# bmerry/mlsgpu

Hardware: AMD Instinct MI355X
Metric: Mvoxels/s evaluated+triangulated (higher is better)
Workload: dtype f32; 1 GPU; cfg3: 512^3 grid, 50000000 splats (uniform), 27 buckets of <= 171 cells per side, octree+MLS+MC end-to-end; bucket_splats_total=52997386, mesh_memory_mb=4096, device_workers=3, batch=8, marching_group=2, mls_variant=culled+matrix-prefilter, counts_cover=the whole cloud

## Files before the change

mlsgpu_amd/csrc/octree.hip:

```cpp
#include "common.hpp"
#include "primitives.hpp"

#include <cstdlib>

using namespace mlsgpu;

struct LevelOffsets
{
    uint32_t v[32];
};

struct mlsgpu_tree
{
    mlsgpu_ctx *ctx = nullptr;
    uint64_t maxLevels = 0, maxSplats = 0;
    uint64_t maxStart = 0, commandsSize = 0;
    uint32_t numLevels = 0;
    DeviceArray<int32_t> dStart, dJumpPos, dCommands;
    DeviceArray<uint32_t> dKeysA, dKeysB, dValsA, dValsB;
    DeviceArray<uint32_t> dHist, dTileSums, dNumEntries;
    DeviceArray<uint32_t> dNodeCounts, dNodeBase;
    DeviceArray<uint32_t> dDigitBase;
    DeviceArray<U3> dNodeTiles;
    HostMailbox entryBox;
    DeviceArray<uint8_t> dSlotMasks;
    DeviceArray<uint64_t> dEntryNotes;
    mlsgpu_splat *dSplats = nullptr;
    bool mutate = true;

    mlsgpu_tree(uint64_t maxLevels, uint64_t maxSplats) : maxLevels(maxLevels), maxSplats(maxSplats)
    {
        maxStart = (uint64_t(1) << (3 * maxLevels)) / 7;
        commandsSize = maxSplats * 8 + std::min(maxStart, 8 * maxSplats) * 2;
    }
    ~mlsgpu_tree() { entryBox.destroy(); }

    template<typename Each>
    int buffers(Each each)
    {
        const uint64_t entries = maxSplats * 8;
        const uint64_t histElems = sortHistElems(entries);
        PROPAGATE(each(dStart, maxStart));
        PROPAGATE(each(dJumpPos, maxStart));
        PROPAGATE(each(dCommands, commandsSize));
        PROPAGATE(each(dKeysA, entries));
        PROPAGATE(each(dKeysB, entries));
        PROPAGATE(each(dValsA, entries));
        PROPAGATE(each(dValsB, entries));
        PROPAGATE(each(dHist, histElems));
        PROPAGATE(each(dTileSums, (uint64_t) scanTiles(std::max(histElems, entries)) + 1));
        PROPAGATE(each(dNumEntries, 1));
        PROPAGATE(each(dSlotMasks, maxSplats));
        PROPAGATE(each(dEntryNotes, maxSplats));
        PROPAGATE(each(dNodeCounts, maxStart));
        PROPAGATE(each(dNodeBase, maxStart));
        PROPAGATE(each(dDigitBase, 257));
        PROPAGATE(each(dNodeTiles, (uint64_t) scanTiles(maxStart) + 1));
        return MLSGPU_OK;
    }
};

namespace
{

__device__ __forceinline__ uint32_t spread3(uint32_t v)
{
    v &= 0x3FFu;
    v = (v | (v << 16)) & 0x030000FFu;
    v = (v | (v << 8)) & 0x0300F00Fu;
    v = (v | (v << 4)) & 0x030C30C3u;
    v = (v | (v << 2)) & 0x09249249u;
    return v;
}
__device__ __forceinline__ uint32_t spreadNext(uint32_t s)
{
    return ((s | ~0x09249249u) + 1u) & 0x09249249u;
}
__device__ __forceinline__ uint32_t makeCode(int x, int y, int z)
{
    return spread3((uint32_t) x) | (spread3((uint32_t) y) << 1) | (spread3((uint32_t) z) << 2);
}
static_assert((0x09249249u & 7u) == 1u, "spread3 keeps bit 0 of a coordinate in bit 0");

__device__ uint32_t makeCodeLoop(int x, int y, int z)
{
    uint32_t ans = 0, scale = 1;
    y <<= 1;
    z <<= 2;
    while (x != 0 || y != 0 || z != 0)
    {
        uint32_t bits = (x & 1) | (y & 2) | (z & 4);
        ans += bits * scale;
        scale <<= 3;
        x >>= 1; y >>= 1; z >>= 1;
    }
    return ans;
}

__device__ __forceinline__ int levelShift(int lox, int loy, int loz, int hix, int hiy, int hiz)
{
    int big = max(max(hix - lox, hiy - loy), hiz - loz);
    return big > 1 ? 32 - __clz(big - 1) : 0;
}

__device__ __forceinline__ float pointBoxDist2(float px, float py, float pz, float lx, float ly, float lz,
                                                float hx, float hy, float hz)
{
    float dx = fmaxf(lx, fminf(hx, px)) - px;
    float dy = fmaxf(ly, fminf(hy, py)) - py;
    float dz = fmaxf(lz, fminf(hz, pz)) - pz;
    return dx * dx + dy * dy + dz * dz;
}

__device__ __forceinline__ int floorToInt(float v)
{
    float f = floorf(v);
    if (!(f > -2147483648.0f)) return INT32_MIN;
    if (!(f < 2147483648.0f)) return INT32_MAX;
    return (int) f;
}

struct EntryParams
{
    mlsgpu_splat *splats;
    int bx, by, bz;
    LevelOffsets levelOffsets;
    int minShift, maxShift;
    uint32_t firstSplat;
    uint32_t mutate;
};

struct EntryPlace
{
    int shift, ilx, ily, ilz;
};

__device__ __forceinline__ uint32_t splatEntries(const EntryParams &P, const float4 pr, uint32_t k[8], EntryPlace *place = nullptr)
{
    const int lox = floorToInt(pr.x - pr.w), loy = floorToInt(pr.y - pr.w), loz = floorToInt(pr.z - pr.w);
    const int hix = floorToInt(pr.x + pr.w), hiy = floorToInt(pr.y + pr.w), hiz = floorToInt(pr.z + pr.w);
    int shift = levelShift(lox, loy, loz, hix, hiy, hiz);
    shift = min(max(shift, P.minShift), P.maxShift);
    const int ilx = max(lox - P.bx, 0) >> shift;
    const int ily = max(loy - P.by, 0) >> shift;
    const int ilz = max(loz - P.bz, 0) >> shift;
    float radius2 = pr.w * pr.w;
    radius2 *= 1.00001f;
    const uint32_t levelOffset = P.levelOffsets.v[shift];
    const int bound = 1 << (P.maxShift - shift);
    if (place != nullptr)
        *place = EntryPlace{shift, ilx, ily, ilz};
    uint32_t mask = 0;
#pragma unroll
    for (int o = 0; o < 8; o++)
    {
        const int ax = ilx + (o & 1), ay = ily + ((o >> 1) & 1), az = ilz + (o >> 2);
        const int blx = (int) ((uint32_t) ax << shift) + P.bx, bhx = (int) ((uint32_t) (ax + 1) << shift) + P.bx;
        const int bly = (int) ((uint32_t) ay << shift) + P.by, bhy = (int) ((uint32_t) (ay + 1) << shift) + P.by;
        const int blz = (int) ((uint32_t) az << shift) + P.bz, bhz = (int) ((uint32_t) (az + 1) << shift) + P.bz;
        bool isect = pointBoxDist2(pr.x, pr.y, pr.z, (float) blx, (float) bly, (float) blz,
                                   (float) bhx, (float) bhy, (float) bhz) < radius2;
        isect = isect && ax < bound && ay < bound && az < bound;
        k[o] = makeCode(ax, ay, az) + levelOffset;
        mask |= (isect ? 1u : 0u) << o;
    }
    return mask;
}

struct EntryCountIn
{
    EntryParams P;
    uint8_t *slotMasks;
    __device__ __forceinline__ uint32_t operator()(uint64_t i) const
    {
        const float4 pr = reinterpret_cast<const float4 *>(P.splats + (i + P.firstSplat))[0];
        uint32_t k[8];
        const uint32_t mask = splatEntries(P, pr, k);
        slotMasks[i] = (uint8_t) mask;
        return (uint32_t) __popc(mask);
    }
};

struct EntryMaskIn
{
    const uint8_t *slotMasks;
    __device__ __forceinline__ uint32_t operator()(uint64_t i) const { return (uint32_t) __popc((uint32_t) slotMasks[i]); }
};

struct EntryWriteOut
{
    EntryParams P;
    const uint8_t *slotMasks;
    uint32_t *keys, *values;
    __device__ __forceinline__ void operator()(uint64_t i, uint32_t pos, uint32_t) const
    {
        const uint32_t gid = (uint32_t) i + P.firstSplat;
        float4 *sp = reinterpret_cast<float4 *>(P.splats + gid);
        const float4 pr = sp[0];
        if (P.mutate)
            reinterpret_cast<float *>(sp)[3] = 1.0f / (pr.w * pr.w);
        const uint32_t mask = slotMasks[i];
        if (mask == 0)
            return;
        const int lox = floorToInt(pr.x - pr.w), loy = floorToInt(pr.y - pr.w), loz = floorToInt(pr.z - pr.w);
        const int hix = floorToInt(pr.x + pr.w), hiy = floorToInt(pr.y + pr.w), hiz = floorToInt(pr.z + pr.w);
        int shift = levelShift(lox, loy, loz, hix, hiy, hiz);
        shift = min(max(shift, P.minShift), P.maxShift);
        const int ilx = max(lox - P.bx, 0) >> shift;
        const int ily = max(loy - P.by, 0) >> shift;
        const int ilz = max(loz - P.bz, 0) >> shift;
        const uint32_t levelOffset = P.levelOffsets.v[shift];
#pragma unroll
        for (int o = 0; o < 8; o++)
            if (mask & (1u << o))
            {
                keys[pos] = makeCode(ilx + (o & 1), ily + ((o >> 1) & 1), ilz + (o >> 2)) + levelOffset;
                values[pos] = gid;
                pos++;
            }
    }
};

enum
{
    ENT_THREADS = 512,
    ENT_PER = 2,
    ENT_TILE = ENT_THREADS * ENT_PER,
    ENT_CAP = 8 * ENT_TILE,
    ENT_BIN_BITS = 8,
    ENT_KEY_BITS = 22,
    ENT_MIN_DIGIT_BITS = 3
};
static_assert(ENT_PER == 1 || ENT_PER == 2, "the splat's place in the tile has 32 - ENT_KEY_BITS bits");

__device__ __forceinline__ uint64_t packNote(uint32_t mask, const EntryPlace &pl)
{
    if (mask == 0)
        return 0;
    const uint32_t lo = mask | (uint32_t) pl.shift << 8 | ((uint32_t) pl.ilx & 0x3FFu) << 13;
    const uint32_t hi = ((uint32_t) pl.ily & 0x3FFu) | ((uint32_t) pl.ilz & 0x3FFu) << 10;
    return (uint64_t) lo | (uint64_t) hi << 32;
}

struct EntryHistArgs
{
    EntryParams P;
    uint64_t *notes;
    uint32_t *hist;
    uint32_t numTiles;
    uint64_t n;
};

__global__ __launch_bounds__(ENT_THREADS) void entryHistKernel(Lanes<EntryHistArgs> lanes, uint32_t digitBits)
{
    const EntryHistArgs &A = lanes.a[blockIdx.y];
    if (blockIdx.x >= A.numTiles)
        return;
    __shared__ uint32_t bins[1 << ENT_BIN_BITS];
    const uint32_t numBins = 1u << digitBits, dmask = numBins - 1;
    for (uint32_t d = threadIdx.x; d < numBins; d += ENT_THREADS)
        bins[d] = 0;
    __syncthreads();
    const uint32_t tile = tileOfWorkgroup(blockIdx.x, A.numTiles);
    const uint64_t i0 = (uint64_t) tile * ENT_TILE + (uint64_t) threadIdx.x * ENT_PER;
    float4 pr[ENT_PER];
#pragma unroll
    for (int s_ = 0; s_ < ENT_PER; s_++)
        pr[s_] = reinterpret_cast<const float4 *>(A.P.splats + ((i0 + s_ < A.n ? i0 + s_ : 0) + A.P.firstSplat))[0];
#pragma unroll
    for (int s_ = 0; s_ < ENT_PER; s_++)
        if (i0 + s_ < A.n)
        {
            uint32_t k[8];
            EntryPlace pl;
            const uint32_t mask = splatEntries(A.P, pr[s_], k, &pl);
            A.notes[i0 + s_] = packNote(mask, pl);
            if (A.P.mutate)
                reinterpret_cast<float *>(A.P.splats + ((i0 + s_) + A.P.firstSplat))[3] = 1.0f / (pr[s_].w * pr[s_].w);
#pragma unroll
            for (int o = 0; o < 8; o++)
                if (mask & (1u << o))
                    atomicAdd(&bins[k[o] & dmask], 1u);
        }
    __syncthreads();
    uint32_t *const hist = A.hist;
    const uint32_t numTiles = A.numTiles;
    for (uint32_t d = threadIdx.x; d < numBins; d += ENT_THREADS)
        hist[(uint64_t) d * numTiles + tile] = bins[d];
}

struct EntryTotalArgs
{
    const uint32_t *digitTotals;
    uint32_t *total;
    uint32_t *digitBase;
};

__global__ __launch_bounds__(256) void entryTotalKernel(Lanes<EntryTotalArgs> lanes, uint32_t count, uint32_t numBins,
                                                        uint32_t *box, uint32_t seq)
{
    __shared__ uint32_t waveTotals[4];
    for (uint32_t k = 0; k < count; k++)
    {
        const uint32_t *const digitTotals = lanes.a[k].digitTotals;
        const uint32_t mine = threadIdx.x < numBins ? digitTotals[threadIdx.x] : 0u;
        const uint32_t incl = waveInclusiveScan(mine);
        if ((threadIdx.x & 63) == 63)
            waveTotals[threadIdx.x >> 6] = incl;
        __syncthreads();
        uint32_t before = 0;
        for (uint32_t w = 0; w < (threadIdx.x >> 6); w++)
            before += waveTotals[w];
        if (threadIdx.x < numBins)
            lanes.a[k].digitBase[threadIdx.x] = before + incl - mine;
        if (threadIdx.x == 0)
        {
            const uint32_t sum = waveTotals[0] + waveTotals[1] + waveTotals[2] + waveTotals[3];
            lanes.a[k].digitBase[numBins] = sum;
            *lanes.a[k].total = sum;
            __hip_atomic_store(box + 1 + k, sum, __ATOMIC_RELAXED, __HIP_MEMORY_SCOPE_SYSTEM);
        }
        __syncthreads();
    }
    if (threadIdx.x == 0)
    {
        __threadfence_system();
        __hip_atomic_store(box, seq, __ATOMIC_RELEASE, __HIP_MEMORY_SCOPE_SYSTEM);
    }
}

struct EntryScatterArgs
{
    EntryParams P;
    const uint64_t *notes;
    const uint32_t *hist;
    const uint32_t *digitTotals;
    uint32_t numTiles;
    uint64_t n;
    uint32_t *keysOut, *valsOut;
    uint32_t idBits;
};

struct NoteKeys
{
    uint32_t x[2], yz[4];
    NoteKeys() = default;
    __device__ __forceinline__ NoteKeys(uint64_t note, const LevelOffsets &levelOffsets)
    {
        const uint32_t lo32 = (uint32_t) note, hi32 = (uint32_t) (note >> 32);
        const uint32_t ilx = (lo32 >> 13) & 0x3FFu, ily = hi32 & 0x3FFu, ilz = (hi32 >> 10) & 0x3FFu;
        const uint32_t levelOffset = levelOffsets.v[(lo32 >> 8) & 0x1Fu];
        const uint32_t sx[2] = {spread3(ilx), spreadNext(spread3(ilx))};
        const uint32_t sy[2] = {spread3(ily), spreadNext(spread3(ily))};
        const uint32_t sz[2] = {spread3(ilz), spreadNext(spread3(ilz))};
        for (uint32_t i = 0; i < 2; i++)
            x[i] = sx[i] << 3;
        for (uint32_t i = 0; i < 4; i++)
            yz[i] = (sy[i & 1] << 4) + (sz[i >> 1] << 5) + (levelOffset << 3);
    }
    __device__ __forceinline__ uint32_t key8(int o) const { return x[o & 1] + yz[o >> 1]; }
};

__global__ __launch_bounds__(ENT_THREADS) __attribute__((amdgpu_waves_per_eu(ENT_PER == 2 ? 6 : 8, 8))) void entryScatterKernel(Lanes<EntryScatterArgs> lanes, uint32_t digitBits)
{
    enum { BINS = 1 << ENT_BIN_BITS, WAVES = ENT_THREADS / 64, GROUPS = ENT_TILE / 64, MAX_ROUNDS = ENT_CAP / ENT_THREADS };
    static_assert(BINS <= ENT_THREADS, "one thread per bin in the scan over the digits");
    const EntryScatterArgs &A = lanes.a[blockIdx.y];
    if (blockIdx.x >= A.numTiles)
        return;
    const EntryParams &P = A.P;
    const uint64_t *const notes = A.notes;
    const uint32_t *const hist = A.hist;
    const uint32_t *const digitTotals = A.digitTotals;
    const uint32_t numTiles = A.numTiles;
    const uint64_t n = A.n;
    uint32_t *const keysOut = A.keysOut, *const valsOut = A.valsOut;
    typedef unsigned long long Word;
    __shared__ union
    {
        Word match[GROUPS][BINS];
        uint32_t ent[ENT_CAP];
    } s;
    static_assert(sizeof(s.match) <= sizeof(s.ent), "the matrix fits the entries' space");
    __shared__ uint32_t sPlace[GROUPS][BINS];
    __shared__ uint32_t tileBase[BINS];
    __shared__ uint32_t waveTotals[WAVES], waveTotalsAll[WAVES];
    const uint32_t numBins = 1u << digitBits, dmask = numBins - 1;
    const uint32_t lane = threadIdx.x & 63, wave = threadIdx.x >> 6;
    for (uint32_t i = threadIdx.x; i < GROUPS * BINS; i += ENT_THREADS)
        (&s.match[0][0])[i] = 0ull;
    const uint32_t tile = tileOfWorkgroup(blockIdx.x, numTiles);
    uint64_t note[ENT_PER];
#pragma unroll
    for (int h = 0; h < ENT_PER; h++)
    {
        const uint64_t i = (uint64_t) tile * ENT_TILE + (uint32_t) h * ENT_THREADS + threadIdx.x;
        note[h] = i < n ? notes[i] : 0ull;
    }
    const uint32_t bin = threadIdx.x;
    const uint32_t totalOfBin = bin < numBins ? digitTotals[bin] : 0u;
    const uint32_t histOfBin = bin < numBins ? hist[(uint64_t) bin * numTiles + tile] : 0u;
    NoteKeys keys[ENT_PER];
#pragma unroll
    for (int h = 0; h < ENT_PER; h++)
        keys[h] = NoteKeys(note[h], P.levelOffsets);
    const uint32_t dmask8 = dmask << 3;
    auto wordOf = [&](int h, int o) { return (keys[h].key8(o) & dmask8) | (((uint32_t) h * WAVES + wave) * (uint32_t) sizeof(s.match[0])); };
    auto matchAt = [&](uint32_t w) { return reinterpret_cast<Word *>(reinterpret_cast<char *>(&s.match[0][0]) + w); };
    auto placeAt = [&](uint32_t w) { return reinterpret_cast<uint32_t *>(reinterpret_cast<char *>(&sPlace[0][0]) + (w >> 1)); };
    __syncthreads();
    const Word bit = 1ull << lane;
#pragma unroll
    for (int h = 0; h < ENT_PER; h++)
#pragma unroll
        for (int o = 0; o < 8; o++)
            if (note[h] & (1u << o))
                atomicOr(matchAt(wordOf(h, o)), bit);
    __syncthreads();
    uint32_t mine = 0, before[GROUPS];
    if (bin < numBins)
    {
#pragma unroll
        for (int g = 0; g < GROUPS; g++)
        {
            before[g] = mine;
            mine += (uint32_t) __popcll(s.match[g][bin]);
        }
    }
    {
        const uint32_t inclMine = waveInclusiveScan(mine), inclAll = waveInclusiveScan(totalOfBin);
        if (lane == 63)
        {
            waveTotals[wave] = inclMine;
            waveTotalsAll[wave] = inclAll;
        }
        __syncthreads();
        uint32_t run = inclMine - mine, base = inclAll - totalOfBin;
        for (uint32_t w = 0; w < wave; w++)
        {
            run += waveTotals[w];
            base += waveTotalsAll[w];
        }
        if (bin < numBins)
        {
#pragma unroll
            for (int g = 0; g < GROUPS; g++)
                sPlace[g][bin] = run + before[g];
            tileBase[bin] = base + histOfBin - run;
        }
    }
    uint32_t tileCount = 0;
#pragma unroll
    for (uint32_t w = 0; w < WAVES; w++)
        tileCount += waveTotals[w];
    if (tileCount == 0)
        return;
    __syncthreads();
    uint32_t dst[ENT_PER][8];
#pragma unroll
    for (int h = 0; h < ENT_PER; h++)
#pragma unroll
        for (int o = 0; o < 8; o++)
            if (note[h] & (1u << o))
            {
                const uint32_t w = wordOf(h, o);
                const Word m = *matchAt(w);
                dst[h][o] = __builtin_amdgcn_mbcnt_hi((uint32_t) (m >> 32), __builtin_amdgcn_mbcnt_lo((uint32_t) m, *placeAt(w)));
            }
    __syncthreads();
#pragma unroll
    for (int h = 0; h < ENT_PER; h++)
    {
        const uint32_t holder = ((uint32_t) h * ENT_THREADS + threadIdx.x) << ENT_KEY_BITS;
#pragma unroll
        for (int o = 0; o < 8; o++)
            if (note[h] & (1u << o))
                s.ent[dst[h][o]] = (keys[h].key8(o) >> 3) | holder;
    }
    __syncthreads();
    const uint32_t idBits = A.idBits;
    const uint32_t tileFirstId = tile * ENT_TILE + (idBits != 0 ? 0u : P.firstSplat);
#pragma unroll
    for (int k = 0; k < MAX_ROUNDS; k++)
    {
        const uint32_t p = threadIdx.x + k * ENT_THREADS;
        if (p < tileCount)
        {
            const uint32_t e = s.ent[p];
            const uint32_t key = e & ((1u << ENT_KEY_BITS) - 1u);
            const uint32_t out = tileBase[key & dmask] + p;
            const uint32_t id = tileFirstId + (e >> ENT_KEY_BITS);
            if (idBits != 0)
                keysOut[out] = (key >> digitBits) << idBits | id;
            else
            {
                keysOut[out] = key;
                valsOut[out] = id;
            }
        }
    }
}

enum { CMD_BINS = 1 << ENT_BIN_BITS };
static_assert(CMD_BINS == PRIM_BLOCK, "one bin and one group begin per thread");

__device__ __forceinline__ void lowPartsOfTile(const uint32_t *lowBase, uint32_t numLow, uint32_t first, uint32_t last,
                                               uint32_t &lowFirst, bool &oneLow, uint32_t &myBegin)
{
    const uint32_t lane = threadIdx.x & 63, wave = threadIdx.x >> 6;
    uint32_t begins[PRIM_WAVES];
#pragma unroll
    for (uint32_t q = 0; q < PRIM_WAVES; q++)
        begins[q] = lowBase[q * 64 + lane];
    uint32_t c0 = 0, c1 = 0;
    myBegin = 0xFFFFFFFFu;
#pragma unroll
    for (uint32_t q = 0; q < PRIM_WAVES; q++)
    {
        const uint32_t begin = q * 64 + lane < numLow ? begins[q] : 0xFFFFFFFFu;
        c0 += (uint32_t) __popcll(__ballot(begin <= first));
        c1 += (uint32_t) __popcll(__ballot(begin <= last));
        if (q == wave)
            myBegin = begin;
    }
    lowFirst = c0 - 1;
    oneLow = c1 == c0;
}

struct CommandHistArgs
{
    const uint32_t *words;
    uint32_t *hist;
    uint32_t n;
    const uint32_t *nDev;
    uint32_t numTiles;
    uint32_t *keyCounts;
    const uint32_t *lowBase;
};

__global__ __launch_bounds__(PRIM_BLOCK) void commandHistKernel(Lanes<CommandHistArgs> lanes, uint32_t shift, uint32_t digitBits,
                                                                uint32_t idBits)
{
    const CommandHistArgs A = lanes.a[blockIdx.y];
    if (blockIdx.x >= A.numTiles)
        return;
    uint32_t n = A.n;
    if (A.nDev != nullptr && *A.nDev < n)
        n = *A.nDev;
    __shared__ uint32_t bins[CMD_BINS];
    __shared__ uint32_t keyBins[KEY_COUNT_SLOTS * CMD_BINS];
    __shared__ uint32_t sLow[CMD_BINS];
    const uint32_t numBins = 1u << digitBits, numLow = 1u << shift;
    const uint32_t lane = threadIdx.x & 63, wave = threadIdx.x >> 6;
    const uint32_t tile = tileOfWorkgroup(blockIdx.x, A.numTiles);
    const uint32_t tileFirst = tile * SORT_TILE;
    const uint32_t tileCount = tileFirst >= n ? 0u : n - tileFirst < SORT_TILE ? n - tileFirst : (uint32_t) SORT_TILE;
    const bool full = tileCount == SORT_TILE;
    const uint32_t at = wave * SORT_WAVE_SPAN + lane;
    const uint32_t *const words = A.words + tileFirst + at;
    uint32_t mine[SORT_ITEMS];
    if (full)
    {
#pragma unroll
        for (int j = 0; j < SORT_ITEMS; j++)
            mine[j] = words[j * 64];
    }
    else
    {
#pragma unroll
        for (int j = 0; j < SORT_ITEMS; j++)
            mine[j] = at + j * 64 < tileCount ? words[j * 64] : 0u;
    }
    uint32_t lowFirst = 0, myBegin;
    bool oneLow = true;
    lowPartsOfTile(A.lowBase, numLow, tileFirst, tileFirst + (tileCount != 0 ? tileCount - 1 : 0u), lowFirst, oneLow, myBegin);
    bins[threadIdx.x] = 0;
    if (!oneLow)
    {
        sLow[threadIdx.x] = myBegin;
#pragma unroll
        for (uint32_t d = threadIdx.x; d < KEY_COUNT_SLOTS * CMD_BINS; d += PRIM_BLOCK)
            keyBins[d] = 0;
    }
    __syncthreads();
    if (full && oneLow)
    {
#pragma unroll
        for (int j = 0; j < SORT_ITEMS; j++)
            atomicAdd(&bins[__builtin_amdgcn_ubfe(mine[j], idBits, digitBits)], 1u);
    }
    else
    {
#pragma unroll
        for (int j = 0; j < SORT_ITEMS; j++)
            if (at + j * 64 < tileCount)
            {
                const uint32_t digit = __builtin_amdgcn_ubfe(mine[j], idBits, digitBits);
                atomicAdd(&bins[digit], 1u);
                if (!oneLow)
                {
                    const uint32_t low = lowPartAt(sLow, lowFirst, numLow, tileFirst + at + j * 64);
                    const uint32_t slot = low - lowFirst;
                    if (slot < KEY_COUNT_SLOTS)
                        atomicAdd(&keyBins[slot * CMD_BINS + digit], 1u);
                    else
                        atomicAdd(&A.keyCounts[(digit << shift) | low], 1u);
                }
            }
    }
    __syncthreads();
    const uint32_t d = threadIdx.x;
    if (d < numBins)
    {
        const uint32_t c = bins[d];
        A.hist[(uint64_t) d * A.numTiles + tile] = c;
        if (oneLow && c != 0)
            atomicAdd(&A.keyCounts[(d << shift) | lowFirst], c);
    }
    if (!oneLow)
#pragma unroll
        for (uint32_t k = threadIdx.x; k < KEY_COUNT_SLOTS * CMD_BINS; k += PRIM_BLOCK)
        {
            const uint32_t c = keyBins[k];
            if (c != 0)
                atomicAdd(&A.keyCounts[((k & (CMD_BINS - 1u)) << shift) | (lowFirst + (k >> ENT_BIN_BITS))], c);
        }
}

struct CommandScatterArgs
{
    const uint32_t *words;
    uint32_t *commands;
    const uint32_t *hist;
    const uint32_t *digitTotals;
    uint32_t n;
    const uint32_t *nDev;
    uint32_t numTiles;
    const uint32_t *keyBase;
    const uint32_t *lowBase;
    uint32_t numKeys;
    uint32_t valueBias;
};

struct CommandTileLds
{
    union
    {
        struct
        {
            unsigned long long match[PRIM_WAVES][CMD_BINS];
            uint32_t run[PRIM_WAVES][CMD_BINS];
        } rank;
        uint32_t tile[SORT_TILE];
    };
    uint32_t tileBase[CMD_BINS];
    uint32_t low[CMD_BINS];
    uint32_t waveTotals[PRIM_WAVES], waveTotalsAll[PRIM_WAVES];
};

template<bool FULL>
__device__ __forceinline__ void commandRounds(CommandTileLds &s, const uint32_t (&word)[SORT_ITEMS], uint32_t (&rank)[SORT_ITEMS],
                                              uint32_t idBits, uint32_t digitBits, uint32_t left)
{
    const uint32_t lane = threadIdx.x & 63, wave = threadIdx.x >> 6;
    unsigned long long *const match = s.rank.match[wave];
    uint32_t *const run = s.rank.run[wave];
    const uint32_t half = lane >> 5, bit = 1u << (lane & 31u);
#pragma unroll
    for (int j = 0; j < SORT_ITEMS; j++)
    {
        const uint32_t digit = __builtin_amdgcn_ubfe(word[j], idBits, digitBits);
        const bool valid = FULL || (uint32_t) j * 64 + lane < left;
        if (valid)
            atomicOr(reinterpret_cast<uint32_t *>(&match[digit]) + half, bit);
        __builtin_amdgcn_wave_barrier();
        rank[j] = 0;
        if (valid)
        {
            const unsigned long long peers = match[digit];
            const uint32_t before = run[digit];
            const uint32_t below = popcBelow(peers);
            rank[j] = before + below;
            if (below == 0)
            {
                run[digit] = before + (uint32_t) __popcll(peers);
                match[digit] = 0ull;
            }
        }
        __builtin_amdgcn_wave_barrier();
    }
}

template<bool FULL>
__device__ __forceinline__ void commandOut(const CommandTileLds &s, uint32_t *commands, uint32_t tileCount, uint32_t idBits,
                                           uint32_t digitBits, uint32_t valueBias)
{
    const uint32_t idMask = (1u << idBits) - 1u;
#pragma unroll
    for (int k = 0; k < SORT_ITEMS; k++)
    {
        const uint32_t p = threadIdx.x + k * PRIM_BLOCK;
        if (FULL || p < tileCount)
        {
            const uint32_t w = s.tile[p];
            commands[s.tileBase[__builtin_amdgcn_ubfe(w, idBits, digitBits)] + p] = (w & idMask) + valueBias;
        }
    }
}

__global__ __launch_bounds__(PRIM_BLOCK) void commandScatterKernel(Lanes<CommandScatterArgs> lanes, uint32_t shift,
                                                                   uint32_t digitBits, uint32_t idBits)
{
    __shared__ CommandTileLds s;
    const CommandScatterArgs A = lanes.a[blockIdx.y];
    if (blockIdx.x >= A.numTiles)
        return;
    uint32_t n = A.n;
    if (A.nDev != nullptr && *A.nDev < n)
        n = *A.nDev;
    const uint32_t tile = tileOfWorkgroup(blockIdx.x, A.numTiles);
    const uint32_t tileFirst = tile * SORT_TILE;
    if (tileFirst >= n)
        return;
    const uint32_t tileCount = n - tileFirst < SORT_TILE ? n - tileFirst : (uint32_t) SORT_TILE;
    const bool full = tileCount == SORT_TILE;
    const uint32_t numBins = 1u << digitBits, numLow = 1u << shift;
    const uint32_t lane = threadIdx.x & 63, wave = threadIdx.x >> 6;
    const uint32_t at = wave * SORT_WAVE_SPAN + lane;
    const uint32_t left = tileCount > wave * SORT_WAVE_SPAN ? tileCount - wave * SORT_WAVE_SPAN : 0u;
    uint32_t lowFirst, myBegin;
    bool oneLow;
    const uint32_t *const words = A.words + tileFirst + at;
    uint32_t word[SORT_ITEMS];
    const uint32_t d = threadIdx.x;
    const bool myBin = d < numBins;
    lowPartsOfTile(A.lowBase, numLow, tileFirst, tileFirst + tileCount - 1, lowFirst, oneLow, myBegin);
    if (full)
    {
#pragma unroll
        for (int j = 0; j < SORT_ITEMS; j++)
            word[j] = words[j * 64];
    }
    else
    {
#pragma unroll
        for (int j = 0; j < SORT_ITEMS; j++)
            word[j] = (uint32_t) j * 64 + lane < left ? words[j * 64] : 0u;
    }
    const uint32_t totalOf = myBin ? A.digitTotals[d] : 0u;
    const uint32_t histOf = myBin ? A.hist[(uint64_t) d * A.numTiles + tile] : 0u;
    const uint32_t myKey = (d << shift) | lowFirst;
    const uint32_t keyBaseOf = A.keyBase[myKey < A.numKeys ? myKey : 0u];
    const uint32_t fold = oneLow ? 1u + keyBaseOf : 0u;
#pragma unroll
    for (uint32_t k = lane; k < CMD_BINS; k += 64)
    {
        s.rank.match[wave][k] = 0ull;
        s.rank.run[wave][k] = 0u;
    }
    s.low[threadIdx.x] = myBegin;
    __builtin_amdgcn_wave_barrier();
    uint32_t rank[SORT_ITEMS];
    if (full)
        commandRounds<true>(s, word, rank, idBits, digitBits, left);
    else
        commandRounds<false>(s, word, rank, idBits, digitBits, left);
    __syncthreads();
    {
        uint32_t c[PRIM_WAVES], mine = 0;
#pragma unroll
        for (int w = 0; w < PRIM_WAVES; w++)
        {
            c[w] = s.rank.run[w][d];
            mine += c[w];
        }
        const uint32_t incl = waveInclusiveScan(mine), inclAll = waveInclusiveScan(totalOf);
        if (lane == 63)
        {
            s.waveTotals[wave] = incl;
            s.waveTotalsAll[wave] = inclAll;
        }
        __syncthreads();
        uint32_t run = incl - mine, base = inclAll - totalOf;
        for (uint32_t w = 0; w < wave; w++)
        {
            run += s.waveTotals[w];
            base += s.waveTotalsAll[w];
        }
        s.tileBase[d] = base + histOf - run + fold;
#pragma unroll
        for (int w = 0; w < PRIM_WAVES; w++)
        {
            s.rank.run[w][d] = run;
            run += c[w];
        }
    }
    __syncthreads();
    uint32_t dst[SORT_ITEMS];
#pragma unroll
    for (int j = 0; j < SORT_ITEMS; j++)
        dst[j] = s.rank.run[wave][__builtin_amdgcn_ubfe(word[j], idBits, digitBits)] + rank[j];
    __syncthreads();
// ... 308 lines not shown
        auto params = [&](uint32_t k) {
            const mlsgpu_tree_build &r = reqs[k];
            return EntryParams{r.dSplats, r.offset[0], r.offset[1], r.offset[2], lo, minShift, maxShift, (uint32_t) r.firstSplat,
                               trees[k]->mutate ? 1u : 0u};
        };
        if (fused)
        {
            const char *stat = "kernel.octree.writeEntries.time";
            auto tilesE = [&](uint32_t a) { return divUp(reqs[act[a]].numSplats, ENT_TILE); };
            auto digitTotals = [&](uint32_t a) { return trees[act[a]]->dHist + (uint64_t) (1u << perPass) * tilesE(a); };
            const auto eh = packLanes<EntryHistArgs>(na, [&](uint32_t a) {
                mlsgpu_tree *t = trees[act[a]];
                return EntryHistArgs{params(act[a]), t->dEntryNotes, t->dHist, tilesE(a), reqs[act[a]].numSplats};
            });
            const auto ds = packLanes<SortDigitScanArgs>(na, [&](uint32_t a) {
                return SortDigitScanArgs{trees[act[a]]->dHist, digitTotals(a), tilesE(a)};
            });
            const auto et = packLanes<EntryTotalArgs>(na, [&](uint32_t a) {
                return EntryTotalArgs{digitTotals(a), trees[act[a]]->dNumEntries, trees[act[a]]->dDigitBase};
            });
            const auto es = packLanes<EntryScatterArgs>(na, [&](uint32_t a) {
                mlsgpu_tree *t = trees[act[a]];
                return EntryScatterArgs{params(act[a]), t->dEntryNotes, t->dHist, digitTotals(a), tilesE(a), reqs[act[a]].numSplats,
                                        t->dKeysB, t->dValsB, idBits};
            });
            const uint32_t maxTiles = mostOfLanes(na, tilesE);
            LAUNCH(ctx, stat, entryHistKernel, dim3(maxTiles, na), dim3(ENT_THREADS), eh, perPass);
            LAUNCH(ctx, stat, (sortDigitScanKernel<uint32_t>), dim3(1u << perPass, na), dim3(PRIM_BLOCK), ds);
            const uint32_t seq = t0->entryBox.reserve();
            LAUNCH(ctx, stat, entryTotalKernel, dim3(1), dim3(256), et, na, 1u << perPass, t0->entryBox.dev, seq);
            LAUNCH(ctx, stat, entryScatterKernel, dim3(maxTiles, na), dim3(ENT_THREADS), es, perPass);
            PROPAGATE(t0->entryBox.wait(ctx->stream));
            for (uint32_t a = 0; a < na; a++)
            {
                mlsgpu_tree *t = trees[act[a]];
                sortN[a] = t0->entryBox.payload()[a];
                sortJobs[a] = SortJob<uint32_t>{t->dKeysB, t->dValsB, t->dKeysA, t->dValsA, sortN[a], t->dHist, t->dNumEntries,
                                                SortResult<uint32_t>{nullptr, nullptr}};
            }
            if (!direct)
                PROPAGATE(radixSortBatch<uint32_t>(ctx, "kernel.octree.sort.time", sortJobs, na, keyBits, false, perPass));
        }
        else
        {
            typedef ScanJob<uint32_t, EntryCountIn, EntryMaskIn, EntryWriteOut> EntryJob;
            EntryJob jobs[MAX_LANES];
            const void *counts[MAX_LANES];
            for (uint32_t a = 0; a < na; a++)
            {
                const uint32_t k = act[a];
                mlsgpu_tree *t = trees[k];
                const EntryParams P = params(k);
                jobs[a] = EntryJob{EntryCountIn{P, t->dSlotMasks}, EntryMaskIn{t->dSlotMasks},
                                   EntryWriteOut{P, t->dSlotMasks, t->dKeysA, t->dValsA}, reqs[k].numSplats, 0u, t->dTileSums,
                                   t->dNumEntries, nullptr};
                counts[a] = t->dNumEntries;
            }
            PROPAGATE((exclusiveScanBatch<uint32_t, EntryCountIn, EntryMaskIn, EntryWriteOut>(
                ctx, "kernel.octree.writeEntries.time", jobs, na)));
            PROPAGATE(t0->entryBox.publishGather(ctx->stream, counts, na, 1));
            PROPAGATE(t0->entryBox.wait(ctx->stream));
            for (uint32_t a = 0; a < na; a++)
            {
                mlsgpu_tree *t = trees[act[a]];
                sortN[a] = t0->entryBox.payload()[a];
                sortJobs[a] = SortJob<uint32_t>{t->dKeysA, t->dValsA, t->dKeysB, t->dValsB, sortN[a], t->dHist, t->dNumEntries,
                                                SortResult<uint32_t>{nullptr, nullptr}};
            }
            PROPAGATE(radixSortBatch<uint32_t>(ctx, "kernel.octree.sort.time", sortJobs, na, keyBits, false));
        }
        if (direct)
        {
            const uint32_t shift = perPass, digitBits = keyBits - perPass;
            const auto h = packLanes<SortHistArgs<uint32_t> >(na, [&](uint32_t a) {
                const SortJob<uint32_t> &j = sortJobs[a];
                return SortHistArgs<uint32_t>{j.keysA, j.dHist, j.n, j.nDev, sortTiles(j.n), trees[act[a]]->dNodeCounts,
                                              trees[act[a]]->dDigitBase, idBits};
            });
            const auto d = packLanes<SortDigitScanArgs>(na, [&](uint32_t a) {
                return SortDigitScanArgs{sortJobs[a].dHist, sortDigitTotals(sortJobs[a]), sortTiles(sortJobs[a].n)};
            });
            const auto ch = packLanes<CommandHistArgs>(na, [&](uint32_t a) {
                const SortJob<uint32_t> &j = sortJobs[a];
                return CommandHistArgs{j.keysA, j.dHist, (uint32_t) j.n, j.nDev, sortTiles(j.n), trees[act[a]]->dNodeCounts,
                                       trees[act[a]]->dDigitBase};
            });
            const uint32_t maxTiles = mostOfLanes(na, [&](uint32_t a) { return sortTiles(sortJobs[a].n); });
            if (maxTiles > 0)
            {
                if (lastPass)
                    LAUNCH(ctx, "kernel.octree.sort.time", commandHistKernel, dim3(maxTiles, na), dim3(PRIM_BLOCK), ch, shift, digitBits,
                           idBits);
                else
                    LAUNCH(ctx, "kernel.octree.sort.time", (sortHistKernel<uint32_t, true>), dim3(maxTiles, na), dim3(PRIM_BLOCK), h,
                           shift, digitBits);
                LAUNCH(ctx, "kernel.octree.sort.time", (sortDigitScanKernel<uint32_t>), dim3(1u << digitBits, na), dim3(PRIM_BLOCK), d);
            }
        }
        else
        {
            typedef ScanJob<uint32_t, IndicatorIn, IndicatorIn, SplatIdsOut> CommandJob;
            CommandJob cj[MAX_LANES];
            for (uint32_t a = 0; a < na; a++)
            {
                mlsgpu_tree *t = trees[act[a]];
                const SortResult<uint32_t> &sorted = sortJobs[a].result;
                const IndicatorIn in{sorted.keys, t->dNumEntries};
                cj[a] = CommandJob{in, in, SplatIdsOut{t->dCommands, t->dStart, t->dJumpPos, sorted.keys, sorted.vals, t->dNumEntries},
                                   sortN[a], 1u, t->dTileSums, (uint32_t *) nullptr, t->dNumEntries};
            }
            PROPAGATE((exclusiveScanBatch<uint32_t, IndicatorIn, IndicatorIn, SplatIdsOut>(ctx, "kernel.octree.scan.time", cj, na)));
        }
    }
    if (direct)
    {
        typedef ScanJob<U3, NodeIn, NodeIn, NodeOut> NodeJob;
        NodeJob nj[MAX_LANES];
        for (uint32_t k = 0; k < count; k++)
        {
            mlsgpu_tree *t = trees[k];
            const NodeIn in{t->dNodeCounts};
            nj[k] = NodeJob{in, in, NodeOut{t->dStart, t->dJumpPos, t->dNodeBase}, numStart, U3{0, 0, 0}, t->dNodeTiles, (U3 *) nullptr,
                            nullptr};
        }
        PROPAGATE((exclusiveScanBatch<U3, NodeIn, NodeIn, NodeOut>(ctx, "kernel.octree.scan.time", nj, count)));
        if (na > 0)
        {
            const uint32_t shift = perPass, digitBits = keyBits - perPass;
            const auto sc = packLanes<SortScatterArgs<uint32_t> >(na, [&](uint32_t a) {
                const SortJob<uint32_t> &j = sortJobs[a];
                mlsgpu_tree *t = trees[act[a]];
                return SortScatterArgs<uint32_t>{j.keysA, j.valsA, (uint32_t *) nullptr, reinterpret_cast<uint32_t *>(t->dCommands.get()), j.dHist,
                                                 sortDigitTotals(j), j.n, j.nDev, sortTiles(j.n), t->dNodeBase, t->dDigitBase, idBits,
                                                 (uint32_t) reqs[act[a]].firstSplat};
            });
            const auto cs = packLanes<CommandScatterArgs>(na, [&](uint32_t a) {
                const SortJob<uint32_t> &j = sortJobs[a];
                mlsgpu_tree *t = trees[act[a]];
                return CommandScatterArgs{j.keysA, reinterpret_cast<uint32_t *>(t->dCommands.get()), j.dHist, sortDigitTotals(j),
                                          (uint32_t) j.n, j.nDev, sortTiles(j.n), t->dNodeBase, t->dDigitBase, numStart,
                                          (uint32_t) reqs[act[a]].firstSplat};
            });
            const uint32_t maxTiles = mostOfLanes(na, [&](uint32_t a) { return sortTiles(sortJobs[a].n); });
            if (maxTiles > 0 && lastPass)
                LAUNCH(ctx, "kernel.octree.sort.time", commandScatterKernel, dim3(maxTiles, na), dim3(PRIM_BLOCK), cs, shift, digitBits,
                       idBits);
            else if (maxTiles > 0)
                LAUNCH(ctx, "kernel.octree.sort.time", (sortScatterKernel<uint32_t, false, 8, true>), dim3(maxTiles, na), dim3(PRIM_BLOCK), sc,
                       shift, digitBits);
        }
    }
    const auto ws = packLanes<WriteStartArgs>(count, [&](uint32_t k) {
        return WriteStartArgs{trees[k]->dStart, trees[k]->dCommands, trees[k]->dJumpPos};
    });
    LAUNCH(ctx, "kernel.octree.writeStart.time", writeStartKernel, dim3(divUp(numStart, 256), count), dim3(256),
           ws, lo, minShift, maxShift, numStart);
    return MLSGPU_OK;
}

MLSGPU_API int mlsgpu_hip_tree_build(mlsgpu_tree *t, mlsgpu_splat *dSplats, uint64_t firstSplat, uint64_t numSplats,
                                     const uint32_t size[3], const int32_t offset[3], uint32_t subsamplingShift)
{
    REQUIRE(t != nullptr && dSplats != nullptr && size != nullptr && offset != nullptr, MLSGPU_ERR_INVALID);
    mlsgpu_tree_build r;
    r.dSplats = dSplats;
    r.firstSplat = firstSplat;
    r.numSplats = numSplats;
    for (int i = 0; i < 3; i++)
    {
        r.size[i] = size[i];
        r.offset[i] = offset[i];
    }
    return treeBuildBatch(&t, &r, 1, subsamplingShift);
}

MLSGPU_API int mlsgpu_hip_tree_build_batch(mlsgpu_tree *const *trees, const mlsgpu_tree_build *builds, uint32_t count,
                                           uint32_t subsamplingShift)
{
    REQUIRE(trees != nullptr && builds != nullptr, MLSGPU_ERR_INVALID);
    REQUIRE(count >= 1 && count <= MLSGPU_MAX_BATCH, MLSGPU_ERR_LENGTH);
    return treeBuildBatch(trees, builds, count, subsamplingShift);
}

MLSGPU_API int mlsgpu_hip_tree_num_entries(mlsgpu_tree *t, uint64_t *out)
{
    REQUIRE(t != nullptr && out != nullptr, MLSGPU_ERR_INVALID);
    HIP_CHECK(hipSetDevice(t->ctx->device));
    uint32_t n = 0;
    HIP_CHECK(hipMemcpyAsync(&n, t->dNumEntries, 4, hipMemcpyDeviceToHost, t->ctx->stream));
    HIP_CHECK(hipStreamSynchronize(t->ctx->stream));
    *out = n;
    return MLSGPU_OK;
}

MLSGPU_API void mlsgpu_hip_tree_clear_splats(mlsgpu_tree *t) { if (t) t->dSplats = nullptr; }
MLSGPU_API const mlsgpu_splat *mlsgpu_hip_tree_splats(const mlsgpu_tree *t) { return t->dSplats; }
MLSGPU_API int mlsgpu_hip_tree_set_mutate(mlsgpu_tree *t, int mutate)
{
    REQUIRE(t != nullptr, MLSGPU_ERR_INVALID);
    t->mutate = mutate != 0;
    return MLSGPU_OK;
}
MLSGPU_API int mlsgpu_hip_tree_mutates(const mlsgpu_tree *t) { return t != nullptr && t->mutate ? 1 : 0; }
MLSGPU_API const int32_t *mlsgpu_hip_tree_commands(const mlsgpu_tree *t) { return t->dCommands; }
MLSGPU_API const int32_t *mlsgpu_hip_tree_start(const mlsgpu_tree *t) { return t->dStart; }
MLSGPU_API uint64_t mlsgpu_hip_tree_commands_size(const mlsgpu_tree *t) { return t->commandsSize; }
MLSGPU_API uint64_t mlsgpu_hip_tree_start_size(const mlsgpu_tree *t) { return t->maxStart; }
MLSGPU_API uint32_t mlsgpu_hip_tree_num_levels(const mlsgpu_tree *t) { return t->numLevels; }

MLSGPU_API int mlsgpu_hip_test_make_code(mlsgpu_ctx *ctx, int x, int y, int z, uint32_t *out)
{
    REQUIRE(ctx != nullptr && out != nullptr, MLSGPU_ERR_INVALID);
    int32_t a[3] = {x, y, z};
    uint32_t loopForm = 0, fast = 0;
    PROPAGATE(runTestHelper(ctx, 0, a, 3, nullptr, 0, &loopForm));
    if (x >= 0 && y >= 0 && z >= 0 && x < 1024 && y < 1024 && z < 1024)
    {
        PROPAGATE(runTestHelper(ctx, 3, a, 3, nullptr, 0, &fast));
        if (fast != loopForm)
            return setError(MLSGPU_ERR_INVALID, "makeCode fast path disagrees with loop form");
    }
    *out = loopForm;
    return MLSGPU_OK;
// ... 23 lines not shown
```

Measured before the change: 10040 Mvoxels/s.

## Use lane-permute level-offset lookup, reorder hist kernel, drop device n clamp

Level offsets are now loaded once into a per-lane register and looked up with ds_bpermute instead of dynamically indexing a kernel-argument array. The aim is to avoid the scratch or scalar loads that dynamic indexing costs in the entry histogram and scatter kernels. The histogram kernel now issues its splat loads before zeroing shared bins, uses a lighter LDS-only barrier, and computes bin atomics without a per-splat branch. The command hist and scatter kernels stop reading the device-side count nDev and use the host n, which is safe only if the host count is never larger than the real entry count.

```diff
diff --git a/mlsgpu_amd/csrc/octree.hip b/mlsgpu_amd/csrc/octree.hip
--- a/mlsgpu_amd/csrc/octree.hip
+++ b/mlsgpu_amd/csrc/octree.hip
@@ -135,7 +135,25 @@
     int shift, ilx, ily, ilz;
 };
 
-__device__ __forceinline__ uint32_t splatEntries(const EntryParams &P, const float4 pr, uint32_t k[8], EntryPlace *place = nullptr)
+struct LaneLevelOffsets
+{
+    uint32_t word;
+    __device__ __forceinline__ explicit LaneLevelOffsets(const LevelOffsets &table) : word(table.v[threadIdx.x & 31u]) {}
+    __device__ __forceinline__ uint32_t operator()(uint32_t level) const
+    {
+        return (uint32_t) __builtin_amdgcn_ds_bpermute((int) (level << 2), (int) word);
+    }
+};
+
+struct TableLevelOffsets
+{
+    const LevelOffsets &table;
+    __device__ __forceinline__ uint32_t operator()(uint32_t level) const { return table.v[level]; }
+};
+
+template<typename LevelOffsetOf>
+__device__ __forceinline__ uint32_t splatEntries(const EntryParams &P, const LevelOffsetOf &levelOffsetOf, const float4 pr,
+                                                 uint32_t k[8], EntryPlace *place = nullptr)
 {
     const int lox = floorToInt(pr.x - pr.w), loy = floorToInt(pr.y - pr.w), loz = floorToInt(pr.z - pr.w);
     const int hix = floorToInt(pr.x + pr.w), hiy = floorToInt(pr.y + pr.w), hiz = floorToInt(pr.z + pr.w);
@@ -146,7 +164,7 @@
     const int ilz = max(loz - P.bz, 0) >> shift;
     float radius2 = pr.w * pr.w;
     radius2 *= 1.00001f;
-    const uint32_t levelOffset = P.levelOffsets.v[shift];
+    const uint32_t levelOffset = levelOffsetOf((uint32_t) shift);
     const int bound = 1 << (P.maxShift - shift);
     if (place != nullptr)
         *place = EntryPlace{shift, ilx, ily, ilz};
@@ -175,7 +193,7 @@
     {
         const float4 pr = reinterpret_cast<const float4 *>(P.splats + (i + P.firstSplat))[0];
         uint32_t k[8];
-        const uint32_t mask = splatEntries(P, pr, k);
+        const uint32_t mask = splatEntries(P, TableLevelOffsets{P.levelOffsets}, pr, k);
         slotMasks[i] = (uint8_t) mask;
         return (uint32_t) __popc(mask);
     }
@@ -251,6 +269,11 @@
     uint64_t n;
 };
 
+__device__ __forceinline__ void ldsBarrier()
+{
+    asm volatile("s_waitcnt lgkmcnt(0)\n\ts_barrier" : : : "memory");
+}
+
 __global__ __launch_bounds__(ENT_THREADS) void entryHistKernel(Lanes<EntryHistArgs> lanes, uint32_t digitBits)
 {
     const EntryHistArgs &A = lanes.a[blockIdx.y];
@@ -258,31 +281,39 @@
         return;
     __shared__ uint32_t bins[1 << ENT_BIN_BITS];
     const uint32_t numBins = 1u << digitBits, dmask = numBins - 1;
+    const uint32_t tile = tileOfWorkgroup(blockIdx.x, A.numTiles);
+    const uint64_t i0 = (uint64_t) tile * ENT_TILE + (uint64_t) threadIdx.x * ENT_PER;
+    const LaneLevelOffsets levelOffsetOf(A.P.levelOffsets);
+    float4 pr[ENT_PER];
+#pragma unroll
+    for (int s_ = 0; s_ < ENT_PER; s_++)
+        pr[s_] = reinterpret_cast<const float4 *>(A.P.splats + ((i0 + s_ < A.n ? i0 + s_ : 0) + A.P.firstSplat))[0];
     for (uint32_t d = threadIdx.x; d < numBins; d += ENT_THREADS)
         bins[d] = 0;
-    __syncthreads();
-    const uint32_t tile = tileOfWorkgroup(blockIdx.x, A.numTiles);
-    const uint64_t i0 = (uint64_t) tile * ENT_TILE + (uint64_t) threadIdx.x * ENT_PER;
-    float4 pr[ENT_PER];
+    ldsBarrier();
+    uint64_t note[ENT_PER];
 #pragma unroll
     for (int s_ = 0; s_ < ENT_PER; s_++)
-        pr[s_] = reinterpret_cast<const float4 *>(A.P.splats + ((i0 + s_ < A.n ? i0 + s_ : 0) + A.P.firstSplat))[0];
+    {
+        uint32_t k[8];
+        EntryPlace pl;
+        const uint32_t all = splatEntries(A.P, levelOffsetOf, pr[s_], k, &pl);
+        const uint32_t mask = i0 + s_ < A.n ? all : 0u;
+        note[s_] = packNote(mask, pl);
+#pragma unroll
+        for (int o = 0; o < 8; o++)
+            if (mask & (1u << o))
+                atomicAdd(&bins[k[o] & dmask], 1u);
+    }
 #pragma unroll
     for (int s_ = 0; s_ < ENT_PER; s_++)
         if (i0 + s_ < A.n)
         {
-            uint32_t k[8];
-            EntryPlace pl;
-            const uint32_t mask = splatEntries(A.P, pr[s_], k, &pl);
-            A.notes[i0 + s_] = packNote(mask, pl);
+            A.notes[i0 + s_] = note[s_];
             if (A.P.mutate)
                 reinterpret_cast<float *>(A.P.splats + ((i0 + s_) + A.P.firstSplat))[3] = 1.0f / (pr[s_].w * pr[s_].w);
-#pragma unroll
-            for (int o = 0; o < 8; o++)
-                if (mask & (1u << o))
-                    atomicAdd(&bins[k[o] & dmask], 1u);
-        }
-    __syncthreads();
+        }
+    ldsBarrier();
     uint32_t *const hist = A.hist;
     const uint32_t numTiles = A.numTiles;
     for (uint32_t d = threadIdx.x; d < numBins; d += ENT_THREADS)
@@ -345,11 +376,11 @@
 {
     uint32_t x[2], yz[4];
     NoteKeys() = default;
-    __device__ __forceinline__ NoteKeys(uint64_t note, const LevelOffsets &levelOffsets)
+    __device__ __forceinline__ NoteKeys(uint64_t note, const LaneLevelOffsets &levelOffsetOf)
     {
         const uint32_t lo32 = (uint32_t) note, hi32 = (uint32_t) (note >> 32);
         const uint32_t ilx = (lo32 >> 13) & 0x3FFu, ily = hi32 & 0x3FFu, ilz = (hi32 >> 10) & 0x3FFu;
-        const uint32_t levelOffset = levelOffsets.v[(lo32 >> 8) & 0x1Fu];
+        const uint32_t levelOffset = levelOffsetOf((lo32 >> 8) & 0x1Fu);
         const uint32_t sx[2] = {spread3(ilx), spreadNext(spread3(ilx))};
         const uint32_t sy[2] = {spread3(ily), spreadNext(spread3(ily))};
         const uint32_t sz[2] = {spread3(ilz), spreadNext(spread3(ilz))};
@@ -390,6 +421,7 @@
     for (uint32_t i = threadIdx.x; i < GROUPS * BINS; i += ENT_THREADS)
         (&s.match[0][0])[i] = 0ull;
     const uint32_t tile = tileOfWorkgroup(blockIdx.x, numTiles);
+    const LaneLevelOffsets levelOffsetOf(P.levelOffsets);
     uint64_t note[ENT_PER];
 #pragma unroll
     for (int h = 0; h < ENT_PER; h++)
@@ -403,7 +435,7 @@
     NoteKeys keys[ENT_PER];
 #pragma unroll
     for (int h = 0; h < ENT_PER; h++)
-        keys[h] = NoteKeys(note[h], P.levelOffsets);
+        keys[h] = NoteKeys(note[h], levelOffsetOf);
     const uint32_t dmask8 = dmask << 3;
     auto wordOf = [&](int h, int o) { return (keys[h].key8(o) & dmask8) | (((uint32_t) h * WAVES + wave) * (uint32_t) sizeof(s.match[0])); };
     auto matchAt = [&](uint32_t w) { return reinterpret_cast<Word *>(reinterpret_cast<char *>(&s.match[0][0]) + w); };
@@ -532,7 +564,6 @@
     const uint32_t *words;
     uint32_t *hist;
     uint32_t n;
-    const uint32_t *nDev;
     uint32_t numTiles;
     uint32_t *keyCounts;
     const uint32_t *lowBase;
@@ -544,9 +575,7 @@
     const CommandHistArgs A = lanes.a[blockIdx.y];
     if (blockIdx.x >= A.numTiles)
         return;
-    uint32_t n = A.n;
-    if (A.nDev != nullptr && *A.nDev < n)
-        n = *A.nDev;
+    const uint32_t n = A.n;
     __shared__ uint32_t bins[CMD_BINS];
     __shared__ uint32_t keyBins[KEY_COUNT_SLOTS * CMD_BINS];
     __shared__ uint32_t sLow[CMD_BINS];
@@ -634,7 +663,6 @@
     const uint32_t *hist;
     const uint32_t *digitTotals;
     uint32_t n;
-    const uint32_t *nDev;
     uint32_t numTiles;
     const uint32_t *keyBase;
     const uint32_t *lowBase;
@@ -715,9 +743,7 @@
     const CommandScatterArgs A = lanes.a[blockIdx.y];
     if (blockIdx.x >= A.numTiles)
         return;
-    uint32_t n = A.n;
-    if (A.nDev != nullptr && *A.nDev < n)
-        n = *A.nDev;
+    const uint32_t n = A.n;
     const uint32_t tile = tileOfWorkgroup(blockIdx.x, A.numTiles);
     const uint32_t tileFirst = tile * SORT_TILE;
     if (tileFirst >= n)
@@ -1192,7 +1218,7 @@
             });
             const auto ch = packLanes<CommandHistArgs>(na, [&](uint32_t a) {
                 const SortJob<uint32_t> &j = sortJobs[a];
-                return CommandHistArgs{j.keysA, j.dHist, (uint32_t) j.n, j.nDev, sortTiles(j.n), trees[act[a]]->dNodeCounts,
+                return CommandHistArgs{j.keysA, j.dHist, (uint32_t) j.n, sortTiles(j.n), trees[act[a]]->dNodeCounts,
                                        trees[act[a]]->dDigitBase};
             });
             const uint32_t maxTiles = mostOfLanes(na, [&](uint32_t a) { return sortTiles(sortJobs[a].n); });
@@ -1248,7 +1274,7 @@
                 const SortJob<uint32_t> &j = sortJobs[a];
                 mlsgpu_tree *t = trees[act[a]];
                 return CommandScatterArgs{j.keysA, reinterpret_cast<uint32_t *>(t->dCommands.get()), j.dHist, sortDigitTotals(j),
-                                          (uint32_t) j.n, j.nDev, sortTiles(j.n), t->dNodeBase, t->dDigitBase, numStart,
+                                          (uint32_t) j.n, sortTiles(j.n), t->dNodeBase, t->dDigitBase, numStart,
                                           (uint32_t) reqs[act[a]].firstSplat};
             });
             const uint32_t maxTiles = mostOfLanes(na, [&](uint32_t a) { return sortTiles(sortJobs[a].n); });
```

Result: no change. 10010 Mvoxels/s (-0.2%).

## Pack splat entry notes into 32-bit Morton codes and inline entry computation

Applied to the files above, without the earlier changes.

Replaces the 64-bit per-splat note (mask, level shift, three 10-bit coordinates) with a 32-bit word holding the mask, a 3-bit level index relative to minShift, and the interleaved Morton code of the node. The histogram kernel now computes entries with a new inlined splatNote that also yields byte offsets for the shared-memory bins. The scatter kernel rebuilds the keys from the code and derives level offsets arithmetically instead of looking them up in a table. This halves note traffic between the two passes and removes the spread step in the scatter, but it depends on the level and code fitting into 32 bits and on the arithmetic level offset matching the table.

```diff
diff --git a/mlsgpu_amd/csrc/octree.hip b/mlsgpu_amd/csrc/octree.hip
--- a/mlsgpu_amd/csrc/octree.hip
+++ b/mlsgpu_amd/csrc/octree.hip
@@ -24,7 +24,7 @@
     DeviceArray<U3> dNodeTiles;
     HostMailbox entryBox;
     DeviceArray<uint8_t> dSlotMasks;
-    DeviceArray<uint64_t> dEntryNotes;
+    DeviceArray<uint32_t> dEntryNotes;
     mlsgpu_splat *dSplats = nullptr;
     bool mutate = true;
 
@@ -51,7 +51,7 @@
         PROPAGATE(each(dTileSums, (uint64_t) scanTiles(std::max(histElems, entries)) + 1));
         PROPAGATE(each(dNumEntries, 1));
         PROPAGATE(each(dSlotMasks, maxSplats));
-        PROPAGATE(each(dEntryNotes, maxSplats));
+        PROPAGATE(each(dEntryNotes, 2 * maxSplats));
         PROPAGATE(each(dNodeCounts, maxStart));
         PROPAGATE(each(dNodeBase, maxStart));
         PROPAGATE(each(dDigitBase, 257));
@@ -233,19 +233,75 @@
 };
 static_assert(ENT_PER == 1 || ENT_PER == 2, "the splat's place in the tile has 32 - ENT_KEY_BITS bits");
 
-__device__ __forceinline__ uint64_t packNote(uint32_t mask, const EntryPlace &pl)
-{
-    if (mask == 0)
-        return 0;
-    const uint32_t lo = mask | (uint32_t) pl.shift << 8 | ((uint32_t) pl.ilx & 0x3FFu) << 13;
-    const uint32_t hi = ((uint32_t) pl.ily & 0x3FFu) | ((uint32_t) pl.ilz & 0x3FFu) << 10;
-    return (uint64_t) lo | (uint64_t) hi << 32;
+enum
+{
+    NOTE_LEVEL_SHIFT = 8,
+    NOTE_LEVEL_BITS = 3,
+    NOTE_CODE_SHIFT = NOTE_LEVEL_SHIFT + NOTE_LEVEL_BITS,
+    NOTE_MAX_LEVELS = (ENT_KEY_BITS - 1) / 3 + 1
+};
+static_assert(NOTE_MAX_LEVELS <= (1 << NOTE_LEVEL_BITS), "the level index of a fused build fits the note's level field");
+static_assert(NOTE_CODE_SHIFT + 3 * (NOTE_MAX_LEVELS - 1) <= 32, "the code of a node inside its level fits the note's word");
+static_assert(ENT_BIN_BITS <= 9, "a first-pass digit is made of the low three bits of every node coordinate");
+
+__device__ __forceinline__ uint32_t levelOffsetOf(const EntryParams &P, int shift)
+{
+    const uint32_t numStart = P.levelOffsets.v[P.maxShift] + 1u;
+    const uint32_t low = 3u * (uint32_t) (P.maxShift - shift + 1);
+    return numStart >> low << low;
+}
+
+__device__ __forceinline__ uint32_t splatNote(const EntryParams &P, const float4 pr, uint32_t (&off4)[8])
+{
+    const int lox = floorToInt(pr.x - pr.w), loy = floorToInt(pr.y - pr.w), loz = floorToInt(pr.z - pr.w);
+    const int hix = floorToInt(pr.x + pr.w), hiy = floorToInt(pr.y + pr.w), hiz = floorToInt(pr.z + pr.w);
+    int shift = levelShift(lox, loy, loz, hix, hiy, hiz);
+    shift = min(max(shift, P.minShift), P.maxShift);
+    const uint32_t il[3] = {(uint32_t) (max(lox - P.bx, 0) >> shift), (uint32_t) (max(loy - P.by, 0) >> shift),
+                            (uint32_t) (max(loz - P.bz, 0) >> shift)};
+    const uint32_t b[3] = {(uint32_t) P.bx, (uint32_t) P.by, (uint32_t) P.bz};
+    const float p[3] = {pr.x, pr.y, pr.z};
+    float radius2 = pr.w * pr.w;
+    radius2 *= 1.00001f;
+    const uint32_t levelOffset = levelOffsetOf(P, shift);
+    const int bound = 1 << (P.maxShift - shift);
+    const uint32_t step = 1u << shift;
+    float d2[3][2];
+    bool in[3][2];
+    uint32_t sp[3][2];
+#pragma unroll
+    for (int a = 0; a < 3; a++)
+    {
+        const uint32_t e0 = (il[a] << shift) + b[a], e1 = e0 + step, e2 = e1 + step;
+        const float f0 = (float) (int) e0, f1 = (float) (int) e1, f2 = (float) (int) e2;
+        const float d0 = fmaxf(f0, fminf(f1, p[a])) - p[a], d1 = fmaxf(f1, fminf(f2, p[a])) - p[a];
+        d2[a][0] = d0 * d0;
+        d2[a][1] = d1 * d1;
+        in[a][0] = (int) il[a] < bound;
+        in[a][1] = (int) (il[a] + 1u) < bound;
+        sp[a][0] = spread3(il[a]);
+        sp[a][1] = spreadNext(sp[a][0]);
+    }
+    uint32_t mask = 0;
+#pragma unroll
+    for (int o = 0; o < 8; o++)
+    {
+        const int dx = o & 1, dy = (o >> 1) & 1, dz = o >> 2;
+        const bool isect = d2[0][dx] + d2[1][dy] + d2[2][dz] < radius2 && in[0][dx] && in[1][dy] && in[2][dz];
+        mask |= (isect ? 1u : 0u) << o;
+    }
+    const uint32_t level4 = levelOffset << 2;
+#pragma unroll
+    for (int o = 0; o < 8; o++)
+        off4[o] = (sp[0][o & 1] << 2) + ((sp[1][(o >> 1) & 1] << 3) + ((sp[2][o >> 2] << 4) + level4));
+    const uint32_t code = sp[0][0] | sp[1][0] << 1 | sp[2][0] << 2;
+    return mask == 0 ? 0u : mask | (uint32_t) (shift - P.minShift) << NOTE_LEVEL_SHIFT | code << NOTE_CODE_SHIFT;
 }
 
 struct EntryHistArgs
 {
     EntryParams P;
-    uint64_t *notes;
+    uint32_t *notes;
     uint32_t *hist;
     uint32_t numTiles;
     uint64_t n;
@@ -257,7 +313,7 @@
     if (blockIdx.x >= A.numTiles)
         return;
     __shared__ uint32_t bins[1 << ENT_BIN_BITS];
-    const uint32_t numBins = 1u << digitBits, dmask = numBins - 1;
+    const uint32_t numBins = 1u << digitBits, dmask4 = (numBins - 1) << 2;
     for (uint32_t d = threadIdx.x; d < numBins; d += ENT_THREADS)
         bins[d] = 0;
     __syncthreads();
@@ -267,22 +323,28 @@
 #pragma unroll
     for (int s_ = 0; s_ < ENT_PER; s_++)
         pr[s_] = reinterpret_cast<const float4 *>(A.P.splats + ((i0 + s_ < A.n ? i0 + s_ : 0) + A.P.firstSplat))[0];
+    uint32_t note[ENT_PER];
+#pragma unroll
+    for (int s_ = 0; s_ < ENT_PER; s_++)
+    {
+        uint32_t off4[8];
+        note[s_] = splatNote(A.P, pr[s_], off4);
+        if (!(i0 + s_ < A.n))
+            note[s_] = 0;
+#pragma unroll
+        for (int o = 0; o < 8; o++)
+            if (note[s_] & (1u << o))
+                atomicAdd(reinterpret_cast<uint32_t *>(reinterpret_cast<char *>(bins) + (off4[o] & dmask4)), 1u);
+    }
+    __syncthreads();
 #pragma unroll
     for (int s_ = 0; s_ < ENT_PER; s_++)
         if (i0 + s_ < A.n)
         {
-            uint32_t k[8];
-            EntryPlace pl;
-            const uint32_t mask = splatEntries(A.P, pr[s_], k, &pl);
-            A.notes[i0 + s_] = packNote(mask, pl);
+            A.notes[i0 + s_] = note[s_];
             if (A.P.mutate)
                 reinterpret_cast<float *>(A.P.splats + ((i0 + s_) + A.P.firstSplat))[3] = 1.0f / (pr[s_].w * pr[s_].w);
-#pragma unroll
-            for (int o = 0; o < 8; o++)
-                if (mask & (1u << o))
-                    atomicAdd(&bins[k[o] & dmask], 1u);
-        }
-    __syncthreads();
+        }
     uint32_t *const hist = A.hist;
     const uint32_t numTiles = A.numTiles;
     for (uint32_t d = threadIdx.x; d < numBins; d += ENT_THREADS)
@@ -332,7 +394,7 @@
 struct EntryScatterArgs
 {
     EntryParams P;
-    const uint64_t *notes;
+    const uint32_t *notes;
     const uint32_t *hist;
     const uint32_t *digitTotals;
     uint32_t numTiles;
@@ -345,14 +407,14 @@
 {
     uint32_t x[2], yz[4];
     NoteKeys() = default;
-    __device__ __forceinline__ NoteKeys(uint64_t note, const LevelOffsets &levelOffsets)
-    {
-        const uint32_t lo32 = (uint32_t) note, hi32 = (uint32_t) (note >> 32);
-        const uint32_t ilx = (lo32 >> 13) & 0x3FFu, ily = hi32 & 0x3FFu, ilz = (hi32 >> 10) & 0x3FFu;
-        const uint32_t levelOffset = levelOffsets.v[(lo32 >> 8) & 0x1Fu];
-        const uint32_t sx[2] = {spread3(ilx), spreadNext(spread3(ilx))};
-        const uint32_t sy[2] = {spread3(ily), spreadNext(spread3(ily))};
-        const uint32_t sz[2] = {spread3(ilz), spreadNext(spread3(ilz))};
+    __device__ __forceinline__ NoteKeys(uint32_t note, const EntryParams &P)
+    {
+        const uint32_t code = note >> NOTE_CODE_SHIFT;
+        const uint32_t level = (note >> NOTE_LEVEL_SHIFT) & ((1u << NOTE_LEVEL_BITS) - 1u);
+        const uint32_t levelOffset = levelOffsetOf(P, P.minShift + (int) level);
+        const uint32_t sx[2] = {code & 0x09249249u, spreadNext(code & 0x09249249u)};
+        const uint32_t sy[2] = {(code >> 1) & 0x09249249u, spreadNext((code >> 1) & 0x09249249u)};
+        const uint32_t sz[2] = {(code >> 2) & 0x09249249u, spreadNext((code >> 2) & 0x09249249u)};
         for (uint32_t i = 0; i < 2; i++)
             x[i] = sx[i] << 3;
         for (uint32_t i = 0; i < 4; i++)
@@ -369,7 +431,7 @@
     if (blockIdx.x >= A.numTiles)
         return;
     const EntryParams &P = A.P;
-    const uint64_t *const notes = A.notes;
+    const uint32_t *const notes = A.notes;
     const uint32_t *const hist = A.hist;
     const uint32_t *const digitTotals = A.digitTotals;
     const uint32_t numTiles = A.numTiles;
@@ -390,12 +452,12 @@
     for (uint32_t i = threadIdx.x; i < GROUPS * BINS; i += ENT_THREADS)
         (&s.match[0][0])[i] = 0ull;
     const uint32_t tile = tileOfWorkgroup(blockIdx.x, numTiles);
-    uint64_t note[ENT_PER];
+    uint32_t note[ENT_PER];
 #pragma unroll
     for (int h = 0; h < ENT_PER; h++)
     {
         const uint64_t i = (uint64_t) tile * ENT_TILE + (uint32_t) h * ENT_THREADS + threadIdx.x;
-        note[h] = i < n ? notes[i] : 0ull;
+        note[h] = i < n ? notes[i] : 0u;
     }
     const uint32_t bin = threadIdx.x;
     const uint32_t totalOfBin = bin < numBins ? digitTotals[bin] : 0u;
@@ -403,7 +465,7 @@
     NoteKeys keys[ENT_PER];
 #pragma unroll
     for (int h = 0; h < ENT_PER; h++)
-        keys[h] = NoteKeys(note[h], P.levelOffsets);
+        keys[h] = NoteKeys(note[h], P);
     const uint32_t dmask8 = dmask << 3;
     auto wordOf = [&](int h, int o) { return (keys[h].key8(o) & dmask8) | (((uint32_t) h * WAVES + wave) * (uint32_t) sizeof(s.match[0])); };
     auto matchAt = [&](uint32_t w) { return reinterpret_cast<Word *>(reinterpret_cast<char *>(&s.match[0][0]) + w); };
```

New measurement: 9830 Mvoxels/s before, 9896 Mvoxels/s after, median of 6. About the same (+0.7%).
